# justinkay/coda

Measured on NVIDIA H100. Metric: acquisition steps/sec (M=256,N=5e5,C=100), higher is better.
Workload: dtype f32

## Files before the change

coda_b200/_native.py:

```python
from __future__ import annotations

import ctypes as C
import os
import sys

from . import build as _build

_LIB = None

OK = 0
VERSION = 202
MAX_WORLD = 16
REC_WORDS = 8
FLAG_NONFINITE_INPUT = 0x01
FLAG_RANGE_INPUT = 0x02
FLAG_NONFINITE_TABLE = 0x04
FLAG_NONFINITE_PI = 0x08
FLAG_NONFINITE_PBEST = 0x10
FLAG_NONFINITE_EIG = 0x20
FLAG_NO_CANDIDATE = 0x40
FLAG_XCHG_TIMEOUT = 0x80
FLAG_NEGATIVE_PROB = 0x100
FLAG_ROWSUM_WARN = 0x200
FLAG_PIPELINE_TIMEOUT = 0x400
# ... 36 lines not shown

PX, PS = C.POINTER(XchgStruct), C.POINTER(StepStruct)

SIGNATURES = {
    "coda_b200_last_error": (C.c_char_p, []),
    "coda_b200_version": (i32, []),
    "coda_b200_sm_count": (i32, []),
    "coda_b200_device_check": (i32, []),
    "coda_b200_set_l2_fetch_granularity": (i32, [i32]),
    "coda_b200_xchg_box_bytes": (sz, [i32, i32, i32, i32]),
    "coda_b200_xchg_alloc": (i32, [sz, C.POINTER(p)]),
    "coda_b200_xchg_free": (i32, [p]),
    "coda_b200_ipc_export": (i32, [p, p]),
    "coda_b200_ipc_open": (i32, [p, C.POINTER(p)]),
    "coda_b200_ipc_close": (i32, [p]),
    "coda_b200_peer_enable": (i32, [i32]),
    "coda_b200_scan_slab": (i32, [p, i64, i32, i64, i32, p, p, p, p, p, p]),
    "coda_b200_confusion_accum": (i32, [p, i64, p, i32, i64, i32, i32, p, p]),
    "coda_b200_confusion_sorted": (i32, [p, i64, p, p, i32, i64, i32, i32, p, p]),
    "coda_b200_init_dirichlets": (i32, [p, p, i32, i32, i32, f64, f64, i32, p, p]),
    "coda_b200_scan_compact": (i32, [p, p, i64, i32, i64, i32, i32, p, p, p, p, p, p]),
    "coda_b200_confusion_compact": (i32, [p, p, i64, p, i32, i64, i32, i32, i32, p, p, p]),
    "coda_b200_pi_full_compact": (i32, [p, p, i64, p, i32, i64, i32, i32, p, p, p, p]),
    "coda_b200_pi_rank1_compact": (i32, [p, p, i64, p, i32, i64, i32, i32, p, f64, i32, p, p, p, p, p]),
    "coda_b200_compact_index_count": (i32, [p, i64, i32, i64, i32, i32, p, p]),
    "coda_b200_compact_index_fill": (i32, [p, p, i64, i32, i64, i32, i32, p, p, p, p]),
    "coda_b200_pi_rank1_index": (i32, [p, p, p, p, i32, i64, i32, p, f64, i32, p, p, p, p, p, p]),
    "coda_b200_pi_full": (i32, [p, i64, p, i32, i64, i32, p, p]),
    "coda_b200_pi_full_tc_ok": (i32, [i32, i64, i32, i64]),
    "coda_b200_pi_full_tc_scratch_bytes": (sz, [i32, i32]),
    "coda_b200_pi_full_tc": (i32, [p, i64, p, i32, i64, i32, p, p, p, p]),
    "coda_b200_pi_reduce": (i32, [p, i64, i32, i32, p, p, p, p]),
    "coda_b200_shadow_build": (i32, [p, i64, i32, i64, i32, p, i32, i64, p, p]),
    "coda_b200_pi_rank1": (i32, [p, p, i32, i64, i32, p, f64, i32, p, p, p, p, i32, i32, p]),
    "coda_b200_scan_slab_x": (i32, [p, i32, i64, i32, i64, i32, p, p, p, p, p, p]),
    "coda_b200_confusion_accum_x": (i32, [p, i32, i64, p, i32, i64, i32, i32, p, p]),
    "coda_b200_confusion_sorted_x": (i32, [p, i32, i64, p, p, i32, i64, i32, i32, p, p]),
    "coda_b200_pi_full_x": (i32, [p, i32, i64, p, i32, i64, i32, p, p]),
    "coda_b200_pi_full_tc_ok_x": (i32, [i32, i32, i64, i32, i64]),
    "coda_b200_pi_full_tc_x": (i32, [p, i32, i64, p, i32, i64, i32, p, p, p, p]),
    "coda_b200_shadow_build_x": (i32, [p, i32, i64, i32, i64, i32, p, i32, i64, p, p]),
    "coda_b200_pi_rank1_x": (i32, [p, i32, p, i32, i64, i32, p, f64, i32, p, p, p, p, i32, i32, p]),
    "coda_b200_tables_scratch_bytes": (sz, [i32, i32]),
    "coda_b200_beta_tables": (i32, [p, p, i32, i32, i32, f64, i32, i32, p, p, p, p, p, p, p, p, p, p]),
    "coda_b200_pair_count": (i32, [p, i32, i64, i32, p, p, p, p]),
    "coda_b200_pair_fill": (i32, [p, i32, i64, i32, p, p, p, p, p, p, p, p, p, p]),
    "coda_b200_pair_rows": (i32, [p, i32, i32, p, p, p, p, p, p, p, p, i32, p, p, p, p, p, p]),
    "coda_b200_pair_rows_tc": (i32, [p, i32, i32, p, p, p, p, p, p, p, i32, p, p, p, p, p, p]),
    "coda_b200_template_gains": (i32, [p, i32, i32, p, p, p, p, p]),
    "coda_b200_eig_blocks": (i32, [i64, i32, i32]),
    "coda_b200_gain_eig": (i32, [p, i64, i32, i32, p, p, p, p, p, p, p, p, p, p, p, i64, i32, p, p, i32, p, p, p, p]),
    "coda_b200_ell_build": (i32, [p, p, p, i64, i32, p, p, p]),
    "coda_b200_row_gains": (i32, [p, p, i64, i32, i32, p, p, p, p, p]),
    "coda_b200_step_select": (i32, [PS, PX, p]),
    "coda_b200_step_merge": (i32, [PS, PX, p]),
    "coda_b200_step_label": (i32, [PS, PX, p]),
    "coda_b200_step_mixture": (i32, [PS, PX, p]),
    "coda_b200_ties": (i32, [p, i64, p, p, i64, p, i32, p, p, p, p]),
    "coda_b200_report_gather": (i32, [p, i32, p, PX, p, p]),
    "coda_b200_mp_entropy": (i32, [p, p, i32, i64, i32, f64, p, p, i32, p, p]),
    "coda_b200_static_scores": (i32, [p, p, i32, i64, i32, p, p, p]),
    "coda_b200_select_blocks": (i32, [i64]),
    "coda_b200_weighted_total": (i32, [p, p, i64, p, p, p]),
    "coda_b200_weighted_draw": (i32, [p, p, i64, p, f64, p, p, p]),
    "coda_b200_select_extreme": (i32, [p, p, i64, i32, p, p, p]),
    "coda_b200_select_kth": (i32, [p, p, i64, p, p, i64, p, p]),
}


class NativeError(RuntimeError):
    pass


def lib_path() -> str:
    return _build.LIB


def load(build_if_missing: bool = True):
    global _LIB
    if _LIB is not None:
        return _LIB
    path = lib_path()
    if build_if_missing and not os.environ.get("CODA_B200_NO_BUILD"):
        try:
            _build.build()
        except Exception as e:
            if not os.path.exists(path):
                raise NativeError(f"cannot build {path}: {e}") from e
            if not _build.is_fresh():
                raise NativeError(f"{path} was built from different sources (build.sha256 does not match csrc/ and "
                                  f"include/) and rebuilding failed: {e}") from e
    if not os.path.exists(path):
        raise NativeError(f"{path} is missing; run `python -m coda_b200.build`")
    if os.environ.get("CODA_B200_NO_BUILD") and not _build.is_fresh():
        sys.stderr.write(f"coda_b200: WARNING: {path} does not match the current sources (CODA_B200_NO_BUILD is set)\n")
    lib = C.CDLL(path)
    for name, (res, args) in SIGNATURES.items():
        fn = getattr(lib, name)
        fn.restype = res
        fn.argtypes = args
    if lib.coda_b200_version() != VERSION:
        raise NativeError(f"{path} reports ABI version {lib.coda_b200_version()}, this binding expects {VERSION}")
    _LIB = lib
    return lib


# ... 16 lines not shown
```

coda_b200/csrc/gain.cu:

```cuda
#include "common.cuh"

#include <stdlib.h>

#define GE_THREADS 384
#define GE_WARPS (GE_THREADS / 32)

struct GainEigArgs {
  const float* U;
  long long N;
  int C, H, Hp, T;
  const int32_t* ent_off;
  const int32_t* heavy_off;
  const int32_t* ent_row;
  const uint16_t* ent_cls;
  const float* ph_cache;
  const float* gain;
  const float* PB;
  const float* m0;
  const float* pi_hat;
  const uint8_t* labeled;
  const uint8_t* disagree;
  long long n_offset;
  float* eig;
  long long* partials;
// ... 179 lines not shown
      for (int k = 0; k < KR; ++k) {
        const int c = lane + 32 * k;
        s += u[k];
        if (c < C) e = fmaf(u[k], g0[c], e);
      }
    } else {
      for (int c = lane; c < C; c += 32) {
        const float v = __ldg(urow + c);
        s += v;
        e = fmaf(v, g0[c], e);
      }
    }
    s = warp_sum(s);
    e = warp_sum(e);
    if (lane == 0) {
      const float v = e / fmaxf(s, 1e-12f);
      a.eig[n] = v;
      if (!isfinite(v)) bad |= CODA_B200_FLAG_NONFINITE_EIG;
      if (!a.labeled[n]) {
        best2_add(bB, v, a.n_offset + n);
        if (a.disagree[n]) {
          best2_add(bA, v, a.n_offset + n);
          ++cntA;
        }
      }
    }
    n = nn; e0 = ne0; e1 = ne1; h0 = nh0; h1 = nh1;
  }
  if (lane == 0) {
    s_v[0][warp] = bA.v; s_i[0][warp] = bA.i; s_v2[0][warp] = bA.v2;
    s_v[1][warp] = bB.v; s_i[1][warp] = bB.i; s_v2[1][warp] = bB.v2;
    s_c[warp] = cntA;
  }
  __syncthreads();
  if (tid == 0) {
    Best2 fa = best2_empty(), fb = best2_empty();
    long long cn = 0;
    for (int w = 0; w < GE_WARPS; ++w) {
      best2_merge(fa, Best2{s_v[0][w], s_i[0][w], s_v2[0][w]});
      best2_merge(fb, Best2{s_v[1][w], s_i[1][w], s_v2[1][w]});
      cn += s_c[w];
    }
    rec_store(a.partials + (size_t)blockIdx.x * REC_W, fa, cn, fb);
  }
  if (bad) atomicOr(a.flags, bad);
}

__device__ __forceinline__ float4 ld_stream4(const float4* p) {
  float4 v;
  asm volatile("ld.global.cs.v4.f32 {%0, %1, %2, %3}, [%4];" : "=f"(v.x), "=f"(v.y), "=f"(v.z), "=f"(v.w) : "l"(p));
  return v;
}

template <int NQ>
__global__ void __launch_bounds__(256) k_row_gains(const float* __restrict__ rows, const uint16_t* __restrict__ row_cls,
                                                   long long nrows, long long T, int H, const float* __restrict__ PB,
                                                   const float* __restrict__ m0, const float* __restrict__ pi_hat,
                                                   float* __restrict__ gain) {
  constexpr int Hp = 128 * NQ;
  constexpr int CH = 32;
  const int warp = threadIdx.x >> 5, lane = threadIdx.x & 31;
  float4 m[NQ], fm[NQ];
#pragma unroll
  for (int q = 0; q < NQ; ++q) {
    const int h = (q * 32 + lane) * 4;
    float4 v = __ldg(reinterpret_cast<const float4*>(m0) + q * 32 + lane);
    if (h + 0 >= H) v.x = 0.f;
    if (h + 1 >= H) v.y = 0.f;
    if (h + 2 >= H) v.z = 0.f;
    if (h + 3 >= H) v.w = 0.f;
    m[q] = v;
    fm[q] = make_float4(ent_term(v.x), ent_term(v.y), ent_term(v.z), ent_term(v.w));
  }
  const long long nchunks = (nrows + CH - 1) / CH;
  for (long long ch = (long long)blockIdx.x * 8 + warp; ch < nchunks; ch += (long long)gridDim.x * 8) {
    const long long p0 = ch * CH;
    const long long p1 = min(nrows, p0 + CH);
    int mycls = 0;
    if (p0 + lane < p1) mycls = (p0 + lane < T) ? (int)((p0 + lane) / (1 + H)) : (int)row_cls[p0 + lane - T];
    for (long long i = p0; i < p1; i += 4) {
      float4 a[4][NQ];
#pragma unroll
      for (int j = 0; j < 4; ++j) {
        const long long r = min(i + j, nrows - 1);
        const float4* rp = reinterpret_cast<const float4*>(rows + (size_t)r * Hp);
#pragma unroll
        for (int q = 0; q < NQ; ++q) a[j][q] = ld_stream4(rp + q * 32 + lane);
      }
#pragma unroll
      for (int j = 0; j < 4; ++j) {
        const long long r = i + j;
        if (r < p1) {
          const int c = __shfl_sync(CODA_FULL, mycls, (int)(r - p0));
          const float pic = __ldg(pi_hat + c);
          const float4* pb = reinterpret_cast<const float4*>(PB + (size_t)c * Hp);
          float g = 0.f;
#pragma unroll
          for (int q = 0; q < NQ; ++q) g += gain4(a[j][q], __ldg(pb + q * 32 + lane), m[q], fm[q], pic);
          g = warp_sum(g);
          if (lane == 0) gain[r] = g;
        }
      }
    }
  }
}

__global__ void __launch_bounds__(256) k_row_gains_any(const float* __restrict__ rows, const uint16_t* __restrict__ row_cls,
                                                       long long nrows, long long T, int H, int Hp, const float* __restrict__ PB,
                                                       const float* __restrict__ m0, const float* __restrict__ pi_hat,
                                                       float* __restrict__ gain) {
  extern __shared__ __align__(16) unsigned char smem_raw[];
  float* m0s = reinterpret_cast<float*>(smem_raw);
  float* fm0 = m0s + Hp;
  for (int h = threadIdx.x; h < Hp; h += blockDim.x) {
    const float m = h < H ? m0[h] : 0.f;
    m0s[h] = m;
    fm0[h] = ent_term(m);
  }
  __syncthreads();
  const int warp = threadIdx.x >> 5, lane = threadIdx.x & 31;
  for (long long r = (long long)blockIdx.x * 8 + warp; r < nrows; r += (long long)gridDim.x * 8) {
    const int c = r < T ? (int)(r / (1 + H)) : (int)row_cls[r - T];
    const float pic = pi_hat[c];
    const float* row = rows + (size_t)r * Hp;
    const float* pb = PB + (size_t)c * Hp;
    float g = 0.f;
    for (int hq = lane * 4; hq < Hp; hq += 128) {
      const float4 ph = ld_stream4(reinterpret_cast<const float4*>(row + hq));
      const float4 p4 = __ldg(reinterpret_cast<const float4*>(pb + hq));
      const float4 m4 = *reinterpret_cast<const float4*>(m0s + hq);
      const float4 f4 = *reinterpret_cast<const float4*>(fm0 + hq);
      g += gain4(ph, p4, m4, f4, pic);
    }
    g = warp_sum(g);
    if (lane == 0) gain[r] = g;
  }
}

extern "C" int coda_b200_row_gains(const float* ph_cache, const uint16_t* row_cls, int64_t n_heavy, int H, int C,
                                   const float* PB, const float* m0, const float* pi_hat, float* gain,
                                   coda_stream_t stream) {
  CODA_CHECK_ARG(ph_cache && PB && m0 && pi_hat && gain && (row_cls || n_heavy == 0), "row_gains: null pointer");
  const int Hp = (H + 31) / 32 * 32;
  const long long T = (long long)C * (1 + H);
  const long long nrows = T + (n_heavy > 0 ? n_heavy : 0);
  const float* rows = ph_cache;
  float* g = gain;
  cudaStream_t st = as_stream(stream);
  if (Hp % 128 == 0 && Hp <= 512) {
    int grid = (int)min((long long)(nrows + 255) / 256, (long long)coda_sm_count() * 6);
    if (grid < 1) grid = 1;
#define LAUNCH_RG(NQ) k_row_gains<NQ><<<grid, 256, 0, st>>>(rows, row_cls, nrows, T, H, PB, m0, pi_hat, g)
    if (Hp == 128) LAUNCH_RG(1);
    else if (Hp == 256) LAUNCH_RG(2);
    else if (Hp == 384) LAUNCH_RG(3);
    else LAUNCH_RG(4);
#undef LAUNCH_RG
    CODA_LAUNCH_OK("k_row_gains");
    return CODA_B200_OK;
  }
  int grid = (int)min((long long)(nrows + 7) / 8, (long long)coda_sm_count() * 8);
  if (grid < 1) grid = 1;
  k_row_gains_any<<<grid, 256, (size_t)2 * Hp * 4, st>>>(rows, row_cls, nrows, T, H, Hp, PB, m0, pi_hat, g);
  CODA_LAUNCH_OK("k_row_gains_any");
  return CODA_B200_OK;
}

template <int KC8, int IT8>
__global__ void __launch_bounds__(256, (IT8 == 1 ? 3 : 2)) k_eig_assemble_g8(GainEigArgs a, int nblocks_rec) {
  extern __shared__ __align__(16) unsigned char smem_raw[];
  float* g0 = reinterpret_cast<float*>(smem_raw);
  __shared__ float s_v[2][8], s_v2[2][8];
  __shared__ long long s_i[2][8], s_c[8];
  const int C = a.C;
  for (int c = threadIdx.x; c < C; c += blockDim.x) g0[c] = a.gain[(size_t)c * (1 + a.H)];
  __syncthreads();
  const int warp = threadIdx.x >> 5, lane = threadIdx.x & 31, g = lane & 7, grp = lane >> 3;
  Best2 bA = best2_empty(), bB = best2_empty();
  long long cntA = 0;
  uint32_t bad = 0;
  const long long per_iter = (long long)gridDim.x * 8 * 4 * IT8;
  for (long long wb = ((long long)blockIdx.x * 8 + warp) * 4 * IT8; wb < a.N; wb += per_iter) {
    const long long nb = wb + grp * IT8;
    int e0[IT8], ne[IT8];
    if (!a.ell_row) {
#pragma unroll
      for (int i = 0; i < IT8; ++i) {
        const long long n = min(nb + i, a.N - 1);
        e0[i] = __ldg(a.ent_off + n);
        ne[i] = __ldg(a.ent_off + n + 1) - e0[i];
      }
    }
    float u[IT8][KC8];
    int er[IT8][4], ec[IT8][4];
#pragma unroll
    for (int i = 0; i < IT8; ++i) {
      const long long n = min(nb + i, a.N - 1);
      const float* urow = a.U + (size_t)n * C;
#pragma unroll
      for (int k = 0; k < KC8; ++k) {
        const int c = g + 8 * k;
        u[i][k] = c < C ? __ldg(urow + c) : 0.f;
      }
#pragma unroll
      for (int j = 0; j < 4; ++j) {
        const int e = g + 8 * j;
        er[i][j] = -1; ec[i][j] = 0;
        if (a.ell_row) {
          if (e < a.ell_k) {
            er[i][j] = __ldg(a.ell_row + (size_t)n * a.ell_k + e);
            ec[i][j] = __ldg(a.ell_cls + (size_t)n * a.ell_k + e);
          }
        } else if (e < ne[i]) {
          er[i][j] = __ldg(a.ent_row + e0[i] + e);
          ec[i][j] = __ldg(a.ent_cls + e0[i] + e);
        }
      }
    }
// ... 222 lines not shown
```

coda_b200/csrc/step.cu:

```cuda
#include "xchg.cuh"
#include "terms.cuh"

#define ST_THREADS 256

__device__ void apply_label(const coda_step_t& a, int t, const int* jv, int* cnt , bool valid) {
  const int H = a.H, C = a.C, tid = threadIdx.x;
  unsigned long long* pz = reinterpret_cast<unsigned long long*>(a.pisum_fx);
  for (int c = tid; c < C; c += ST_THREADS) pz[c] = 0ull;
  int32_t* hdr = a.terms;
  R1Term* terms = reinterpret_cast<R1Term*>(a.terms + 2);
  if (!valid) {
    if (tid == 0) { hdr[0] = 0; hdr[1] = -1; }
    return;
  }
  for (int h = tid; h < H; h += ST_THREADS) {
    a.jvec[h] = jv[h];
    a.D[((size_t)h * C + t) * C + jv[h]] += a.lr;
  }
  __shared__ int s_tp, s_m, s_total;
  __shared__ int wtot[ST_THREADS / 32];
  for (int c = tid; c < C; c += ST_THREADS) cnt[c] = 0;
  __syncthreads();
  for (int h = tid; h < H; h += ST_THREADS) atomicAdd(&cnt[jv[h]], 1);
  __syncthreads();
// ... 317 lines not shown
  if (x.world > 1) xch_done(x, XCH_PISUM, ep);
}

static int check_step(const coda_step_t* st, const char* who) {
  CODA_CHECK_ARG(st, "%s: null state", who);
  CODA_CHECK_ARG(st->H >= 1 && st->H <= 1024 && st->C >= 2 && st->C <= 4096 && st->N >= 1, "%s: bad dims", who);
  CODA_CHECK_ARG(st->flags, "%s: flags missing", who);
  return CODA_B200_OK;
}

static size_t select_smem(int H, int C) { return 64 + 2 * (size_t)xch_align16((uint32_t)H * 2) + (size_t)H * 4 + (size_t)C * 4; }

static int launch_select(const coda_step_t* st, const coda_xchg_t* x, int pick, coda_stream_t stream) {
  if (int rc = check_step(st, "step_select")) return rc;
  CODA_CHECK_ARG(st->partials && st->nblocks >= 1 && st->bestrec, "step_select: selection buffers missing");
  if (pick) {
    CODA_CHECK_ARG(st->hard && st->labeled && st->D && st->jvec && st->sel && st->terms && st->pisum_fx && st->labels_global &&
                       st->step_ctr,
                   "step_select: null pointer");
    CODA_CHECK_ARG(2 * st->H <= R1_MAXT && (reinterpret_cast<uintptr_t>(st->terms) & 7) == 0, "step_select: bad terms buffer");
  }
  XchgView v;
  if (int rc = xchg_view_from(x, &v)) return rc;
  k_step_select<<<1, ST_THREADS, select_smem(st->H, st->C), as_stream(stream)>>>(*st, v, pick);
  CODA_LAUNCH_OK("k_step_select");
  return CODA_B200_OK;
}

extern "C" int coda_b200_step_select(const coda_step_t* st, const coda_xchg_t* x, coda_stream_t stream) {
  return launch_select(st, x, 1, stream);
}
extern "C" int coda_b200_step_merge(const coda_step_t* st, const coda_xchg_t* x, coda_stream_t stream) {
  return launch_select(st, x, 0, stream);
}

extern "C" int coda_b200_step_label(const coda_step_t* st, const coda_xchg_t* x, coda_stream_t stream) {
  if (int rc = check_step(st, "step_label")) return rc;
  CODA_CHECK_ARG(st->hard && st->labeled && st->D && st->jvec && st->sel && st->terms && st->pisum_fx, "step_label: null pointer");
  CODA_CHECK_ARG(2 * st->H <= R1_MAXT && (reinterpret_cast<uintptr_t>(st->terms) & 7) == 0, "step_label: bad terms buffer");
  XchgView v;
  if (int rc = xchg_view_from(x, &v)) return rc;
  const size_t smem = 16 + (size_t)xch_align16((uint32_t)st->H * 2) + (size_t)st->H * 4 + (size_t)st->C * 4;
  k_step_label<<<1, ST_THREADS, smem, as_stream(stream)>>>(*st, v);
  CODA_LAUNCH_OK("k_step_label");
  return CODA_B200_OK;
}

extern "C" int coda_b200_step_mixture(const coda_step_t* st, const coda_xchg_t* x, coda_stream_t stream) {
  if (int rc = check_step(st, "step_mixture")) return rc;
  CODA_CHECK_ARG(st->pisum_fx && st->PB && st->pi_hat && st->m0 && st->h_before && st->best_model, "step_mixture: null pointer");
  XchgView v;
  if (int rc = xchg_view_from(x, &v)) return rc;
  const size_t smem = (size_t)xch_align16((uint32_t)st->C * 8) + (size_t)st->C * 4;
  k_step_mixture<<<1, ST_THREADS, smem, as_stream(stream)>>>(*st, v);
  CODA_LAUNCH_OK("k_step_mixture");
  return CODA_B200_OK;
}

__global__ void __launch_bounds__(256) k_ties(const float* __restrict__ eig, long long N,
                                              const uint8_t* __restrict__ labeled,
                                              const uint8_t* __restrict__ disagree, long long n_offset,
                                              const long long* __restrict__ best, int cap,
                                              long long* __restrict__ tie_hdr, long long* __restrict__ tie_idx,
                                              float* __restrict__ tie_val) {
  const bool useA = best[2] > 0;
  const float bv = __int_as_float((int)(useA ? best[0] : best[3]));
  for (long long n = (long long)blockIdx.x * blockDim.x + threadIdx.x; n < N;
       n += (long long)gridDim.x * blockDim.x) {
    if (labeled[n]) continue;
    if (useA && !disagree[n]) continue;
    const float e = eig[n];
    if (isclose_best(e, bv)) {
      const long long g = n_offset + n;
      unsigned long long k = atomicAdd(reinterpret_cast<unsigned long long*>(tie_hdr), 1ull);
      atomicMin(tie_hdr + 1, g);
      if (k < (unsigned long long)cap) {
        tie_idx[k] = g;
        tie_val[k] = e;
      }
    }
  }
}

__global__ void k_ties_reset(long long* tie_hdr) {
  tie_hdr[0] = 0;
  tie_hdr[1] = IDX_NONE;
}

extern "C" int coda_b200_ties(const float* eig, int64_t N, const uint8_t* labeled, const uint8_t* disagree,
                              int64_t n_offset, const int64_t* best, int cap, int64_t* tie_hdr, int64_t* tie_idx,
                              float* tie_val, coda_stream_t stream) {
  CODA_CHECK_ARG(eig && labeled && disagree && best && tie_hdr && tie_idx && tie_val, "ties: null pointer");
  int grid = (int)min((long long)(N + 255) / 256, (long long)coda_sm_count() * 4);
  if (grid < 1) grid = 1;
  k_ties_reset<<<1, 1, 0, as_stream(stream)>>>(reinterpret_cast<long long*>(tie_hdr));
  k_ties<<<grid, 256, 0, as_stream(stream)>>>(eig, N, labeled, disagree, n_offset,
                                              reinterpret_cast<const long long*>(best), cap,
                                              reinterpret_cast<long long*>(tie_hdr),
                                              reinterpret_cast<long long*>(tie_idx), tie_val);
  CODA_LAUNCH_OK("k_ties");
  return CODA_B200_OK;
}

__global__ void __launch_bounds__(ST_THREADS) k_report_gather(const long long* __restrict__ rep, int rep_words,
                                                              long long* __restrict__ rep_all, XchgView x,
                                                              uint32_t* __restrict__ flags) {
  if (x.world <= 1) {
// ... 28 lines not shown
```

coda_b200/engine.py:

```python
from __future__ import annotations

import contextlib
import math
import os

import numpy as np
import torch

from . import _native as nat

_CONST_SLOTS = {}
_CONST_TERMS = 3584


def _acquire_const_slot(dev_index, H):
    per = (2 * H + 63) // 64 * 64
    used = _CONST_SLOTS.setdefault(dev_index, set())
    for s in range(_CONST_TERMS // per):
        if s not in used:
            used.add(s)
            return s
    return -1


# ... 64 lines not shown
        self.Hp = (H + 31) // 32 * 32
        self.W = self.Hp // 32
        self.P = 256
        self.T = Cc * (1 + H)
        self.mode = mode
        self.world = int(world)
        self.n_offset = int(n_offset)
        self.n_global = int(n_global if n_global is not None else N)
        self.lr = float(learning_rate)
        self.hyp_w = float(hyp_w)
        self.prior_strength = 1 - alpha
        self.multiplier = float(multiplier)
        self.uniform_prior = bool(uniform_prior)
        if H > 1024:
            raise NotImplementedError("coda_b200: H > 1024 models is not supported yet")
        if Cc > 4096:
            raise NotImplementedError("coda_b200: C > 4096 classes is not supported yet")
        self.fx_shift = max(8, min(40, 62 - math.ceil(math.log2(self.n_global + 1))))
        self.counters = {"launches": 0}
        self.overlap = os.environ.get("CODA_B200_OVERLAP", "1") != "0"
        self.use_graph = os.environ.get("CODA_B200_GRAPH", "1") != "0"
        self.profile, self.profile_only = None, None
        self.xchg = None
        self._mailbox = None
        self._pi_tc, self._pi_scratch = None, None
        self.cidx = None
        self.stream = torch.cuda.Stream(device=self.dev) if own_stream else None
        self.side = torch.cuda.Stream(device=self.dev)
        self.ev_fork, self.ev_join, self.ev_tables = torch.cuda.Event(), torch.cuda.Event(), torch.cuda.Event()
        self.graphs = {}
        self.labels_ptr = None
        self.const_slot = _acquire_const_slot(self.dev.index, H) if os.environ.get("CODA_B200_R1_CONST", "1") != "0" else -1
        with self._on():
            self._alloc_static()

    @contextlib.contextmanager
    def _on(self):
        with torch.cuda.device(self.dev):
            if self.stream is not None:
                with torch.cuda.stream(self.stream):
                    yield
            else:
                yield

    def _cur(self):
        return torch.cuda.current_stream(self.dev)

    def _s(self):
        return self._cur().cuda_stream

    def sync(self):
        (self.stream or torch.cuda.current_stream(self.dev)).synchronize()

    def _call(self, name, *args, n=1):
        prof = self.profile
        key = name[:-2] if name.endswith("_x") else name
        if prof is not None and (self.profile_only is None or key in self.profile_only):
            st = self._cur()
            e0, e1 = torch.cuda.Event(enable_timing=True), torch.cuda.Event(enable_timing=True)
            e0.record(st)
            rc = getattr(self.lib, name)(*args)
            e1.record(st)
            prof.setdefault(key, []).append((e0, e1))
        else:
            rc = getattr(self.lib, name)(*args)
        nat.check(rc, name)
        self.counters["launches"] += n

    def start_profile(self, only=None):
        self.profile, self.profile_only = {}, (set(only) if only else None)

    def stop_profile(self):
        torch.cuda.synchronize(self.dev)
        out = {}
        for k, v in (self.profile or {}).items():
            ts = [a.elapsed_time(b) for a, b in v]
            out[k] = (len(ts), float(sum(ts)), float(max(ts)))
        self.profile = None
        return out

    def _slab_call(self, name, *args, n=1):
        if self.fmt == nat.SLAB_F32:
            self._call(name, _ptr(self.preds), *args, n=n)
        else:
            self._call(name + "_x", _ptr(self.preds), self.fmt, *args, n=n)

    def _z(self, shape, dtype):
        return torch.zeros(shape, dtype=dtype, device=self.dev)

    def _e(self, shape, dtype):
        return torch.empty(shape, dtype=dtype, device=self.dev)

    def _alloc_static(self):
        H, N, C, Hp, P = self.H, self.N, self.C, self.Hp, self.P
        self.hard = self._e((N, H), torch.int16)
        self.pseudo = self._e((N,), torch.int32)
        self.disagree = self._e((N,), torch.uint8)
        self.labeled = self._z((N,), torch.uint8)
        self.conf_buf = self._z((H * C * C + H * C,), torch.int64)
        self.conf_fx = self.conf_buf[: H * C * C].view(H, C, C)
        self.conf_rest = self.conf_buf[H * C * C:].view(H, C) if self.compact is not None else None
        self.D = self._e((H, C, C), torch.float32)
        self.U = self._e((N * C + 4,), torch.float32)[: N * C].view(N, C)
        self.pisum = self._z((C,), torch.int64)
        self.grid = torch.linspace(1e-6, 1 - 1e-6, P).to(self.dev)
        self.dL = self._e((C, H, P), torch.float32)
        self.G0T = self._z((C, P, Hp), torch.float32)
        self.G1T = self._z((C, P, Hp), torch.float32)
        self.PB = self._z((C, Hp), torch.float32)
# ... 149 lines not shown
                       self.K, _ptr(dt), _ptr(rs), _ptr(self.U), s, n=3)
            del dt, rs
        else:
            self._pi_full()
        self._call("coda_b200_pi_reduce", _ptr(self.U), N, C, self.fx_shift, None, _ptr(self.pisum),
                   _ptr(self.flags), s)

    def _pi_full(self):
        H, N, C, s = self.H, self.N, self.C, self._s()
        if self._pi_tc is None:
            want = os.environ.get("CODA_B200_PI_FULL", "tc") != "simt"
            if self.fmt == nat.SLAB_F32:
                self._pi_tc = bool(want and self.lib.coda_b200_pi_full_tc_ok(H, N, C, self.model_stride)
                                   and self.preds.data_ptr() % 16 == 0)
            else:
                tc32 = bool(self.lib.coda_b200_pi_full_tc_ok(H, N, C, N * C))
                ok = bool(self.lib.coda_b200_pi_full_tc_ok_x(self.fmt, H, N, C, self.model_stride))
                if want and tc32 and not ok:
                    raise NotImplementedError(f"coda_b200: the tensor-core marginal pass cannot read this "
                                              f"{self.preds.dtype} slab (C={C}); its fp32 widening would take it")
                self._pi_tc = bool(want and tc32)
            if self._pi_tc:
                self._pi_scratch = self._e((int(self.lib.coda_b200_pi_full_tc_scratch_bytes(H, C)),), torch.uint8)
        if self._pi_tc:
            self._slab_call("coda_b200_pi_full_tc", self.model_stride, _ptr(self.D), H, N, C, _ptr(self.U),
                            _ptr(self._pi_scratch), _ptr(self.flags), s, n=2)
        else:
            self._slab_call("coda_b200_pi_full", self.model_stride, _ptr(self.D), H, N, C, _ptr(self.U), s)

    def _build_rows(self):
        H, N, C, W, T, s = self.H, self.N, self.C, self.W, self.T, self._s()
        ent_cnt = self._e((N,), torch.int32)
        heavy_cnt = self._e((N,), torch.int32)
        cls_heavy = self._z((C,), torch.int32)
        self._call("coda_b200_pair_count", _ptr(self.hard), H, N, C, _ptr(ent_cnt), _ptr(heavy_cnt), _ptr(cls_heavy), s)
        heavy = cls_heavy.cpu().numpy().astype(np.int64)
        n_ent = int(ent_cnt.sum(dtype=torch.int64).item())
        self.n_heavy = int(heavy.sum())
        self.n_entries = n_ent
        self.max_entries = int(ent_cnt.max().item())
        per_cls = 1 + H + heavy
        cls_base = np.zeros(C + 1, dtype=np.int64)
        np.cumsum(per_cls, out=cls_base[1:])
        self.npairs = int(cls_base[-1])
        if self.npairs >= 2 ** 31 or n_ent >= 2 ** 31:
            raise NotImplementedError("coda_b200: more than 2^31 rows in one shard")
        self.ent_off = self._z((N + 1,), torch.int32)
        self.heavy_off = self._z((N + 1,), torch.int32)
        torch.cumsum(ent_cnt, 0, out=self.ent_off[1:])
        torch.cumsum(heavy_cnt, 0, out=self.heavy_off[1:])
        del ent_cnt, heavy_cnt
        self.cls_base_host = cls_base
        self.cls_base = torch.from_numpy(cls_base).to(self.dev)
        def make_tiles(width):
            nt = (per_cls + width - 1) // width
            tile_off = np.zeros(C + 1, dtype=np.int64)
            np.cumsum(nt, out=tile_off[1:])
            cls_of_tile = np.repeat(np.arange(C, dtype=np.int64), nt)
            k_in_cls = np.arange(int(tile_off[-1]), dtype=np.int64) - tile_off[cls_of_tile]
            start = cls_base[cls_of_tile] + width * k_in_cls
            cnt = np.minimum(width, per_cls[cls_of_tile] - width * k_in_cls)
            tiles = np.stack([cls_of_tile, start, cnt, np.zeros_like(cnt)], axis=1).astype(np.int32)
            return tile_off, int(nt.max()), torch.from_numpy(tiles).to(self.dev)
        width = 128 if self.use_tc else 32
        tile_off, self.max_cls_tiles, self.tiles = make_tiles(width)
        self.tile_off_host = tile_off
        self.tile_off = torch.from_numpy(tile_off).to(self.dev)
        self.ntiles = int(tile_off[-1])
        self.ent_row = self._e((max(1, n_ent),), torch.int32)
        self.ent_cls = self._e((max(1, n_ent),), torch.int16)
        self.zmask = self._e((self.npairs, W), torch.int32)
        self.row_of = self._e((self.npairs,), torch.int32)
        self.row_cls = self._e((max(1, self.n_heavy),), torch.int16)
        cursor = self._z((C,), torch.int32)
        self._call("coda_b200_pair_fill", _ptr(self.hard), H, N, C, _ptr(self.ent_off), _ptr(self.heavy_off),
                   _ptr(self.cls_base), _ptr(cursor), _ptr(self.ent_row), _ptr(self.ent_cls), _ptr(self.zmask),
                   _ptr(self.row_of), _ptr(self.row_cls), s, n=2)
        self.ell_row, self.ell_cls, self.ell_k = None, None, 0
        if 0 < self.max_entries <= 32 and C <= 128:
            self.ell_k = (self.max_entries + 3) // 4 * 4
            self.ell_row = self._e((N, self.ell_k), torch.int32)
            self.ell_cls = self._e((N, self.ell_k), torch.int16)
            self._call("coda_b200_ell_build", _ptr(self.ent_off), _ptr(self.ent_row), _ptr(self.ent_cls), N, self.ell_k,
                       _ptr(self.ell_row), _ptr(self.ell_cls), s)
        self.gain = self._z((self.npairs,), torch.float32)
        self.fused_score = os.environ.get("CODA_B200_FUSED_SCORE", "0") == "1"
        self.ph_cache = None
        if self.mode == "incremental":
            need = self.npairs * self.Hp * 4
            free, _total = torch.cuda.mem_get_info(self.dev)
            if need + (2 << 30) > free + torch.cuda.memory_reserved(self.dev) - torch.cuda.memory_allocated(self.dev):
                import warnings
                warnings.warn(f"coda_b200: row cache of {need / 2 ** 30:.1f} GiB does not fit "
                              f"({free / 2 ** 30:.1f} GiB free); falling back to mode='recompute'")
                self.mode = "recompute"
            else:
                self.ph_cache = self._e((self.npairs, self.Hp), torch.float32)

    def shadow_reserve(self) -> int:
        env = os.environ.get("CODA_B200_SHADOW_RESERVE_GB")
        if env is not None:
            return int(float(env) * 2 ** 30)
        return 4 * self.N * self.C + (1 << 30)

    def _build_shadow(self, left: int = 1, total: int = 1):
        self.shadow, self.slot_of_model, self.n_shadow, self.shadow_cs = None, None, 0, 0
# ... 22 lines not shown
            return
        slot = torch.full((H,), -1, dtype=torch.int32, device=self.dev)
        if self.esz == 4:
            self.shadow = self._e((S + ne, C, cs), torch.float32)
            self.ens_shadow = self.shadow[S] if ne else None
        else:
            self.shadow = self._e((S, C, cs), self.preds.dtype) if S > 0 else None
            self.ens_shadow = self._e((C, cs), torch.float32) if ne else None
        if S > 0:
            order = order[:S].contiguous()
            slot[order.long()] = torch.arange(S, dtype=torch.int32, device=self.dev)
            self._slab_call("coda_b200_shadow_build", self.model_stride, H, N, C, _ptr(order), S, cs,
                            _ptr(self.shadow), self._s())
        if ne:
            first = torch.zeros(1, dtype=torch.int32, device=self.dev)
            self._call("coda_b200_shadow_build", _ptr(self.ens), N * C, 1, N, C, _ptr(first), 1, cs,
                       _ptr(self.ens_shadow), self._s())
        self.slot_of_model, self.n_shadow, self.shadow_cs = slot, S, cs

    def _tables(self, lo, hi, sel=False):
        H, C, s = self.H, self.C, self._s()
        if sel:
            self._call("coda_b200_beta_tables", _ptr(self.D), _ptr(self.grid), H, C, self.P, self.hyp_w, 0, 1,
                       _ptr(self.sel), _ptr(self.scratch), _ptr(self.dL), _ptr(self.G0T), _ptr(self.G1T),
                       _ptr(self.PB), _ptr(self.dLb), _ptr(self.Gb), _ptr(self.flags), s, n=3)
            return
        for b0 in range(lo, hi, self.table_batch):
            b1 = min(hi, b0 + self.table_batch)
            self._call("coda_b200_beta_tables", _ptr(self.D), _ptr(self.grid), H, C, self.P, self.hyp_w, b0, b1, None,
                       _ptr(self.scratch), _ptr(self.dL), _ptr(self.G0T), _ptr(self.G1T), _ptr(self.PB),
                       _ptr(self.dLb), _ptr(self.Gb), _ptr(self.flags), s, n=3)

    def _mixture(self):
        self._call("coda_b200_step_mixture", self.st, self._x(), self._s())

    def _pair_rows(self, tile_lo, tile_hi, gains=True, sel=False):
        tail = (_ptr(self.PB), _ptr(self.m0) if gains else None, _ptr(self.pi_hat) if gains else None, self.H,
                _ptr(self.ph_cache), _ptr(self.gain) if gains else None, _ptr(self.sel) if sel else None,
                _ptr(self.tile_off) if sel else None, _ptr(self.flags), self._s())
        if self.use_tc:
            self._call("coda_b200_pair_rows_tc", _ptr(self.tiles), int(tile_lo), int(tile_hi), _ptr(self.zmask),
                       _ptr(self.row_of), _ptr(self.dLb), _ptr(self.Gb), *tail)
        else:
            self._call("coda_b200_pair_rows", _ptr(self.tiles), int(tile_lo), int(tile_hi), _ptr(self.zmask),
                       _ptr(self.row_of), _ptr(self.dL), _ptr(self.G0T), _ptr(self.G1T), *tail)

    def _score(self):
        if self.scored:
            return
        if self.mode == "incremental":
            if not self.cache_valid:
                self._pair_rows(0, self.ntiles, gains=False)
                self.cache_valid = True
            if self.pending:
                self._cur().wait_event(self.ev_join)
                self.pending = False
            if self.fused_score:
                self._call("coda_b200_template_gains", _ptr(self.ph_cache), self.H, self.C, _ptr(self.PB), _ptr(self.m0),
                           _ptr(self.pi_hat), _ptr(self.gain), self._s())
            else:
                self._call("coda_b200_row_gains", _ptr(self.ph_cache), _ptr(self.row_cls), self.n_heavy, self.H, self.C,
                           _ptr(self.PB), _ptr(self.m0), _ptr(self.pi_hat), _ptr(self.gain), self._s())
        else:
            if self.pending:
                self._cur().wait_event(self.ev_join)
                self.pending = False
            self._pair_rows(0, self.ntiles)
        self._call("coda_b200_gain_eig", _ptr(self.U), self.N, self.C, self.H, _ptr(self.ent_off), _ptr(self.heavy_off),
                   _ptr(self.ent_row), _ptr(self.ent_cls), _ptr(self.ph_cache) if self.fused_score else None,
                   _ptr(self.gain), _ptr(self.PB), _ptr(self.m0), _ptr(self.pi_hat), _ptr(self.labeled),
                   _ptr(self.disagree), self.n_offset, self.max_entries, _ptr(self.ell_row), _ptr(self.ell_cls),
                   self.ell_k, _ptr(self.eig), _ptr(self.partials), _ptr(self.flags), self._s())
        self.scored = True

    def _post_label(self):
        H, N, C, s = self.H, self.N, self.C, self._s()
        self.scored = False
        self.reported = False
        if self.mode == "recompute_all":
            self._pi_full()
            self._call("coda_b200_pi_reduce", _ptr(self.U), N, C, self.fx_shift, None, _ptr(self.pisum), _ptr(self.flags), s)
            self._tables(0, C)
            self._mixture()
            return
        main = self._cur()
        refresh_rows = self.mode == "incremental" and self.cache_valid
        fork = self.overlap
        if fork:
            self.ev_fork.record(main)
            self.side.wait_event(self.ev_fork)
            ctx = torch.cuda.stream(self.side)
        else:
            ctx = contextlib.nullcontext()
        with ctx:
            self._tables(0, 1, sel=True)
            if fork:
                self.ev_tables.record(self.side)
            if refresh_rows:
                self._pair_rows(0, self.max_cls_tiles, gains=False, sel=True)
            if fork:
                self.ev_join.record(self.side)
        if self.compact is not None and self.cidx is not None:
            ix = self.cidx
            self._call("coda_b200_pi_rank1_index", _ptr(ix["off"]), _ptr(ix["ent"]), _ptr(ix["rest"]), _ptr(self.jvec), H, N, C,
                       _ptr(self.sel), self.lr, self.fx_shift, _ptr(self.terms), _ptr(ix["delta"]), _ptr(self.U),
                       _ptr(self.pisum), _ptr(self.flags), s, n=2)
        elif self.compact is not None:
            cs = self.compact
            self._call("coda_b200_pi_rank1_compact", _ptr(cs.ids), _ptr(cs.probs), self.model_stride, _ptr(self.ens), H, N,
                       C, self.K, _ptr(self.sel), self.lr, self.fx_shift, _ptr(self.terms), _ptr(self.U),
                       _ptr(self.pisum), _ptr(self.flags), s)
        else:
            ens = _ptr(self.ens) if self.fmt == nat.SLAB_F32 else self._ens_base()
            self._slab_call("coda_b200_pi_rank1", ens, H, N, C, _ptr(self.sel), self.lr,
                            self.fx_shift, _ptr(self.terms), _ptr(self.U), _ptr(self.pisum), _ptr(self.flags),
# ... 279 lines not shown
```

include/coda_b200.h:

```cpp
#ifndef CODA_B200_H
#define CODA_B200_H

#include <stddef.h>
#include <stdint.h>

#ifdef __cplusplus
extern "C" {
#endif

#define CODA_B200_VERSION 202
#define CODA_B200_NODES 256
#define CODA_B200_MAX_WORLD 16
#define CODA_B200_REC_WORDS 8

#define CODA_B200_OK 0
#define CODA_B200_EINVAL (-1)
#define CODA_B200_ECUDA (-2)

#define CODA_B200_FLAG_NONFINITE_INPUT 0x01u
#define CODA_B200_FLAG_RANGE_INPUT 0x02u
#define CODA_B200_FLAG_NONFINITE_TABLE 0x04u
#define CODA_B200_FLAG_NONFINITE_PI 0x08u
#define CODA_B200_FLAG_NONFINITE_PBEST 0x10u
#define CODA_B200_FLAG_NONFINITE_EIG 0x20u
// ... 87 lines not shown
                                int H, int64_t N, int C, int K, int fx_shift, int64_t* conf_fx, int64_t* conf_rest,
                                coda_stream_t stream);
int coda_b200_pi_full_compact(const uint16_t* ids, const float* probs, int64_t model_stride, const float* D, int H,
                              int64_t N, int C, int K, float* DT_scratch, float* RS_scratch, float* U,
                              coda_stream_t stream);
int coda_b200_pi_rank1_compact(const uint16_t* ids, const float* probs, int64_t model_stride, const float* ens, int H,
                               int64_t N, int C, int K, const int64_t* sel, double lr, int fx_shift,
                               const int32_t* terms, float* U, int64_t* pisum_fx, uint32_t* flags,
                               coda_stream_t stream);

int coda_b200_compact_index_count(const uint16_t* ids, int64_t model_stride, int H, int64_t N, int C, int K,
                                  int64_t* counts, coda_stream_t stream);
int coda_b200_compact_index_fill(const uint16_t* ids, const float* probs, int64_t model_stride, int H, int64_t N, int C,
                                 int K, int64_t* cursor, void* entries, float* rest_sum, coda_stream_t stream);
int coda_b200_pi_rank1_index(const int64_t* offsets, const void* entries, const float* rest_sum, const int32_t* jvec,
                             int H, int64_t N, int C, const int64_t* sel, double lr, int fx_shift, const int32_t* terms,
                             int64_t* delta, float* U, int64_t* pisum_fx, uint32_t* flags, coda_stream_t stream);

size_t coda_b200_tables_scratch_bytes(int H, int ncls);
int coda_b200_beta_tables(const float* D, const float* grid_x, int H, int C, int P, double hyp_w, int cls_lo,
                          int cls_hi, const int64_t* sel, void* scratch, float* dL ,
                          float* G0T , float* G1T , float* PB , void* dLb,
                          void* Gb, uint32_t* flags, coda_stream_t stream);

int coda_b200_pair_count(const uint16_t* hard, int H, int64_t N, int C, int32_t* ent_cnt ,
                         int32_t* heavy_cnt , int32_t* cls_heavy , coda_stream_t stream);
int coda_b200_pair_fill(const uint16_t* hard, int H, int64_t N, int C, const int32_t* ent_off ,
                        const int32_t* heavy_off , const int64_t* cls_base ,
                        int32_t* cls_cursor , int32_t* ent_row, uint16_t* ent_cls,
                        uint32_t* zmask , int32_t* row_of ,
                        uint16_t* row_cls , coda_stream_t stream);
int coda_b200_pair_rows(const int32_t* tiles, int tile_lo, int tile_hi, const uint32_t* zmask, const int32_t* row_of,
                        const float* dL, const float* G0T, const float* G1T, const float* PB, const float* m0,
                        const float* pi_hat, int H, float* ph_cache, float* gain, const int64_t* sel ,
                        const int64_t* tile_off , uint32_t* flags, coda_stream_t stream);
int coda_b200_pair_rows_tc(const int32_t* tiles128, int tile_lo, int tile_hi, const uint32_t* zmask,
                           const int32_t* row_of, const void* dLb, const void* Gb, const float* PB, const float* m0,
                           const float* pi_hat, int H, float* ph_cache, float* gain, const int64_t* sel,
                           const int64_t* tile_off, uint32_t* flags, coda_stream_t stream);
int coda_b200_template_gains(const float* ph_cache, int H, int C, const float* PB, const float* m0,
                             const float* pi_hat, float* gain , coda_stream_t stream);

int coda_b200_eig_blocks(int64_t N, int H, int C);
int coda_b200_gain_eig(const float* U, int64_t N, int C, int H, const int32_t* ent_off, const int32_t* heavy_off,
                       const int32_t* ent_row, const uint16_t* ent_cls, const float* ph_cache, const float* gain,
                       const float* PB, const float* m0, const float* pi_hat, const uint8_t* labeled,
                       const uint8_t* disagree, int64_t n_offset, int max_entries, const int32_t* ell_row,
                       const uint16_t* ell_cls, int ell_k, float* eig, int64_t* partials, uint32_t* flags,
                       coda_stream_t stream);
int coda_b200_ell_build(const int32_t* ent_off, const int32_t* ent_row, const uint16_t* ent_cls, int64_t N, int K,
                        int32_t* ell_row , uint16_t* ell_cls , coda_stream_t stream);
int coda_b200_row_gains(const float* ph_cache, const uint16_t* row_cls, int64_t n_heavy, int H, int C,
                        const float* PB, const float* m0, const float* pi_hat, float* gain, coda_stream_t stream);

typedef struct coda_step {
  int H, C;
  int64_t N, n_offset;
  int fx_shift;
  float lr;
  const uint16_t* hard;
  uint8_t* labeled;
  float* D;
  int32_t* jvec;
  int64_t* sel;
  int32_t* terms;
  const int32_t* slot_of_model;
  int64_t shadow_off, shadow_col_stride, model_stride;
  int64_t ens_off, ens_col_stride;
  int have_ens;
  int compact_k;
  int64_t* pisum_fx;
  const float* PB;
  float* pi_hat;
  float* m0;
  float* h_before;
  int64_t* best_model;
  const int64_t* partials;
  int nblocks;
  const float* eig;
  int64_t* bestrec;
  const int64_t* labels_global;
  int64_t* hist_idx;
  float* hist_q;
  int32_t* hist_tie;
  int64_t hist_cap;
  int64_t* step_ctr;
  uint32_t* flags;
} coda_step_t;

int coda_b200_step_select(const coda_step_t* st, const coda_xchg_t* x, coda_stream_t stream);
int coda_b200_step_merge(const coda_step_t* st, const coda_xchg_t* x, coda_stream_t stream);
int coda_b200_step_label(const coda_step_t* st, const coda_xchg_t* x, coda_stream_t stream);
int coda_b200_step_mixture(const coda_step_t* st, const coda_xchg_t* x, coda_stream_t stream);

int coda_b200_ties(const float* eig, int64_t N, const uint8_t* labeled, const uint8_t* disagree, int64_t n_offset,
                   const int64_t* best , int cap, int64_t* tie_hdr , int64_t* tie_idx,
                   float* tie_val, coda_stream_t stream);
int coda_b200_report_gather(const int64_t* rep, int rep_words, int64_t* rep_all, const coda_xchg_t* x,
                            uint32_t* flags, coda_stream_t stream);


int coda_b200_mp_entropy(const uint16_t* hard, const float* posterior , int H, int64_t N, int C, double gamma,
                         const uint8_t* labeled, const uint8_t* disagree, int mask_agreeing, float* ent,
                         coda_stream_t stream);
int coda_b200_static_scores(const uint16_t* hard, const float* ens, int H, int64_t N, int C, float* at_score,
                            float* vma_score, coda_stream_t stream);
// ... 15 lines not shown
```

Before: 661.0.

## Split row gains so unaffected classes compute before the pending pair-row join

Row-gain scoring is split into two launches. The first covers every class except the one just labelled and runs before waiting on the side-stream join event. After the join, a second launch recomputes only the labelled class's rows through a row_of/cls_base index. This lets most of the gain work overlap the pending pair-row refresh instead of waiting for it, at the cost of an extra launch and indirect row addressing. The mixture kernel is also launched with high stream priority via cudaLaunchKernelEx, and the grid sizing for the vectorized row kernel now scales with span rather than being capped by SM count.

```diff
diff --git a/coda_b200/_native.py b/coda_b200/_native.py
--- a/coda_b200/_native.py
+++ b/coda_b200/_native.py
@@ -112,6 +112,8 @@
     "coda_b200_gain_eig": (i32, [p, i64, i32, i32, p, p, p, p, p, p, p, p, p, p, p, i64, i32, p, p, i32, p, p, p, p]),
     "coda_b200_ell_build": (i32, [p, p, p, i64, i32, p, p, p]),
     "coda_b200_row_gains": (i32, [p, p, i64, i32, i32, p, p, p, p, p]),
+    "coda_b200_row_gains_except": (i32, [p, p, i64, i32, i32, p, p, p, p, p, p]),
+    "coda_b200_row_gains_class": (i32, [p, p, p, i64, i32, i32, p, p, p, p, p, p]),
     "coda_b200_step_select": (i32, [PS, PX, p]),
     "coda_b200_step_merge": (i32, [PS, PX, p]),
     "coda_b200_step_label": (i32, [PS, PX, p]),
diff --git a/coda_b200/csrc/gain.cu b/coda_b200/csrc/gain.cu
--- a/coda_b200/csrc/gain.cu
+++ b/coda_b200/csrc/gain.cu
@@ -255,14 +255,33 @@
   return v;
 }
 
+struct RowSet {
+  const long long* sel;
+  const int32_t* row_of;
+  const long long* cls_base;
+};
+
+__device__ __forceinline__ void row_set_range(const RowSet& s, long long nrows, long long& p_lo, long long& p_hi,
+                                              int& skip, int& t) {
+  p_lo = 0; p_hi = nrows; skip = -1; t = 0;
+  if (s.sel) {
+    t = (int)s.sel[1];
+    if (s.row_of) { p_lo = s.cls_base[t]; p_hi = s.cls_base[t + 1]; }
+    else skip = t;
+  }
+}
+
 template <int NQ>
 __global__ void __launch_bounds__(256) k_row_gains(const float* __restrict__ rows, const uint16_t* __restrict__ row_cls,
                                                    long long nrows, long long T, int H, const float* __restrict__ PB,
                                                    const float* __restrict__ m0, const float* __restrict__ pi_hat,
-                                                   float* __restrict__ gain) {
+                                                   RowSet rs, float* __restrict__ gain) {
   constexpr int Hp = 128 * NQ;
   constexpr int CH = 32;
   const int warp = threadIdx.x >> 5, lane = threadIdx.x & 31;
+  long long p_lo, p_hi;
+  int skip, t;
+  row_set_range(rs, nrows, p_lo, p_hi, skip, t);
   float4 m[NQ], fm[NQ];
 #pragma unroll
   for (int q = 0; q < NQ; ++q) {
@@ -275,26 +294,42 @@
     m[q] = v;
     fm[q] = make_float4(ent_term(v.x), ent_term(v.y), ent_term(v.z), ent_term(v.w));
   }
-  const long long nchunks = (nrows + CH - 1) / CH;
+  const long long nchunks = (p_hi - p_lo + CH - 1) / CH;
   for (long long ch = (long long)blockIdx.x * 8 + warp; ch < nchunks; ch += (long long)gridDim.x * 8) {
-    const long long p0 = ch * CH;
-    const long long p1 = min(nrows, p0 + CH);
-    int mycls = 0;
-    if (p0 + lane < p1) mycls = (p0 + lane < T) ? (int)((p0 + lane) / (1 + H)) : (int)row_cls[p0 + lane - T];
-    for (long long i = p0; i < p1; i += 4) {
+    const long long p0 = p_lo + ch * CH;
+    const long long p1 = min(p_hi, p0 + CH);
+    int myrow = (int)(p0 + lane);
+    int mycls = t;
+    if (p0 + lane < p1) {
+      if (rs.row_of) myrow = rs.row_of[p0 + lane];
+      else mycls = (p0 + lane < T) ? (int)((p0 + lane) / (1 + H)) : (int)row_cls[p0 + lane - T];
+    }
+    const int n = (int)(p1 - p0);
+    for (int i = 0; i < n; i += 4) {
       float4 a[4][NQ];
+      int rj[4], cj[4];
 #pragma unroll
       for (int j = 0; j < 4; ++j) {
-        const long long r = min(i + j, nrows - 1);
-        const float4* rp = reinterpret_cast<const float4*>(rows + (size_t)r * Hp);
-#pragma unroll
-        for (int q = 0; q < NQ; ++q) a[j][q] = ld_stream4(rp + q * 32 + lane);
+        const int l = min(i + j, n - 1);
+        rj[j] = __shfl_sync(CODA_FULL, myrow, l);
+        cj[j] = __shfl_sync(CODA_FULL, mycls, l);
       }
 #pragma unroll
       for (int j = 0; j < 4; ++j) {
-        const long long r = i + j;
-        if (r < p1) {
-          const int c = __shfl_sync(CODA_FULL, mycls, (int)(r - p0));
+        const float4* rp = reinterpret_cast<const float4*>(rows + (size_t)rj[j] * Hp);
+        if (cj[j] != skip) {
+#pragma unroll
+          for (int q = 0; q < NQ; ++q) a[j][q] = ld_stream4(rp + q * 32 + lane);
+        } else {
+#pragma unroll
+          for (int q = 0; q < NQ; ++q) a[j][q] = make_float4(0.f, 0.f, 0.f, 0.f);
+        }
+      }
+#pragma unroll
+      for (int j = 0; j < 4; ++j) {
+        const int r = rj[j];
+        if (i + j < n && cj[j] != skip) {
+          const int c = cj[j];
           const float pic = __ldg(pi_hat + c);
           const float4* pb = reinterpret_cast<const float4*>(PB + (size_t)c * Hp);
           float g = 0.f;
@@ -311,7 +346,7 @@
 __global__ void __launch_bounds__(256) k_row_gains_any(const float* __restrict__ rows, const uint16_t* __restrict__ row_cls,
                                                        long long nrows, long long T, int H, int Hp, const float* __restrict__ PB,
                                                        const float* __restrict__ m0, const float* __restrict__ pi_hat,
-                                                       float* __restrict__ gain) {
+                                                       RowSet rs, float* __restrict__ gain) {
   extern __shared__ __align__(16) unsigned char smem_raw[];
   float* m0s = reinterpret_cast<float*>(smem_raw);
   float* fm0 = m0s + Hp;
@@ -321,9 +356,14 @@
     fm0[h] = ent_term(m);
   }
   __syncthreads();
+  long long p_lo, p_hi;
+  int skip, t;
+  row_set_range(rs, nrows, p_lo, p_hi, skip, t);
   const int warp = threadIdx.x >> 5, lane = threadIdx.x & 31;
-  for (long long r = (long long)blockIdx.x * 8 + warp; r < nrows; r += (long long)gridDim.x * 8) {
-    const int c = r < T ? (int)(r / (1 + H)) : (int)row_cls[r - T];
+  for (long long p = p_lo + (long long)blockIdx.x * 8 + warp; p < p_hi; p += (long long)gridDim.x * 8) {
+    const long long r = rs.row_of ? (long long)rs.row_of[p] : p;
+    const int c = rs.row_of ? t : (r < T ? (int)(r / (1 + H)) : (int)row_cls[r - T]);
+    if (c == skip) continue;
     const float pic = pi_hat[c];
     const float* row = rows + (size_t)r * Hp;
     const float* pb = PB + (size_t)c * Hp;
@@ -340,10 +380,9 @@
   }
 }
 
-extern "C" int coda_b200_row_gains(const float* ph_cache, const uint16_t* row_cls, int64_t n_heavy, int H, int C,
-                                   const float* PB, const float* m0, const float* pi_hat, float* gain,
-                                   coda_stream_t stream) {
-  CODA_CHECK_ARG(ph_cache && PB && m0 && pi_hat && gain && (row_cls || n_heavy == 0), "row_gains: null pointer");
+static int row_gains_launch(const float* ph_cache, const uint16_t* row_cls, int64_t n_heavy, int H, int C,
+                            const float* PB, const float* m0, const float* pi_hat, RowSet rs, long long span,
+                            float* gain, coda_stream_t stream) {
   const int Hp = (H + 31) / 32 * 32;
   const long long T = (long long)C * (1 + H);
   const long long nrows = T + (n_heavy > 0 ? n_heavy : 0);
@@ -351,9 +390,9 @@
   float* g = gain;
   cudaStream_t st = as_stream(stream);
   if (Hp % 128 == 0 && Hp <= 512) {
-    int grid = (int)min((long long)(nrows + 255) / 256, (long long)coda_sm_count() * 6);
+    int grid = (int)((span + 255) / 256);
     if (grid < 1) grid = 1;
-#define LAUNCH_RG(NQ) k_row_gains<NQ><<<grid, 256, 0, st>>>(rows, row_cls, nrows, T, H, PB, m0, pi_hat, g)
+#define LAUNCH_RG(NQ) k_row_gains<NQ><<<grid, 256, 0, st>>>(rows, row_cls, nrows, T, H, PB, m0, pi_hat, rs, g)
     if (Hp == 128) LAUNCH_RG(1);
     else if (Hp == 256) LAUNCH_RG(2);
     else if (Hp == 384) LAUNCH_RG(3);
@@ -362,11 +401,41 @@
     CODA_LAUNCH_OK("k_row_gains");
     return CODA_B200_OK;
   }
-  int grid = (int)min((long long)(nrows + 7) / 8, (long long)coda_sm_count() * 8);
+  int grid = (int)min((long long)(span + 7) / 8, (long long)coda_sm_count() * 8);
   if (grid < 1) grid = 1;
-  k_row_gains_any<<<grid, 256, (size_t)2 * Hp * 4, st>>>(rows, row_cls, nrows, T, H, Hp, PB, m0, pi_hat, g);
+  k_row_gains_any<<<grid, 256, (size_t)2 * Hp * 4, st>>>(rows, row_cls, nrows, T, H, Hp, PB, m0, pi_hat, rs, g);
   CODA_LAUNCH_OK("k_row_gains_any");
   return CODA_B200_OK;
+}
+
+extern "C" int coda_b200_row_gains(const float* ph_cache, const uint16_t* row_cls, int64_t n_heavy, int H, int C,
+                                   const float* PB, const float* m0, const float* pi_hat, float* gain,
+                                   coda_stream_t stream) {
+  CODA_CHECK_ARG(ph_cache && PB && m0 && pi_hat && gain && (row_cls || n_heavy == 0), "row_gains: null pointer");
+  const long long nrows = (long long)C * (1 + H) + (n_heavy > 0 ? n_heavy : 0);
+  return row_gains_launch(ph_cache, row_cls, n_heavy, H, C, PB, m0, pi_hat, RowSet{nullptr, nullptr, nullptr}, nrows,
+                          gain, stream);
+}
+
+extern "C" int coda_b200_row_gains_except(const float* ph_cache, const uint16_t* row_cls, int64_t n_heavy, int H,
+                                          int C, const float* PB, const float* m0, const float* pi_hat,
+                                          const int64_t* sel, float* gain, coda_stream_t stream) {
+  CODA_CHECK_ARG(ph_cache && PB && m0 && pi_hat && gain && sel && (row_cls || n_heavy == 0),
+                 "row_gains_except: null pointer");
+  const long long nrows = (long long)C * (1 + H) + (n_heavy > 0 ? n_heavy : 0);
+  return row_gains_launch(ph_cache, row_cls, n_heavy, H, C, PB, m0, pi_hat,
+                          RowSet{reinterpret_cast<const long long*>(sel), nullptr, nullptr}, nrows, gain, stream);
+}
+
+extern "C" int coda_b200_row_gains_class(const float* ph_cache, const int32_t* row_of, const int64_t* cls_base,
+                                         int64_t max_cls_rows, int H, int C, const float* PB, const float* m0,
+                                         const float* pi_hat, const int64_t* sel, float* gain, coda_stream_t stream) {
+  CODA_CHECK_ARG(ph_cache && row_of && cls_base && PB && m0 && pi_hat && gain && sel, "row_gains_class: null pointer");
+  CODA_CHECK_ARG(max_cls_rows >= 1, "row_gains_class: max_cls_rows=%lld", (long long)max_cls_rows);
+  return row_gains_launch(ph_cache, nullptr, 0, H, C, PB, m0, pi_hat,
+                          RowSet{reinterpret_cast<const long long*>(sel), row_of,
+                                 reinterpret_cast<const long long*>(cls_base)},
+                          max_cls_rows, gain, stream);
 }
 
 template <int KC8, int IT8>
diff --git a/coda_b200/csrc/step.cu b/coda_b200/csrc/step.cu
--- a/coda_b200/csrc/step.cu
+++ b/coda_b200/csrc/step.cu
@@ -393,7 +393,19 @@
   XchgView v;
   if (int rc = xchg_view_from(x, &v)) return rc;
   const size_t smem = (size_t)xch_align16((uint32_t)st->C * 8) + (size_t)st->C * 4;
-  k_step_mixture<<<1, ST_THREADS, smem, as_stream(stream)>>>(*st, v);
+  int prio_lo = 0, prio_hi = 0;
+  CODA_CUDA_OK(cudaDeviceGetStreamPriorityRange(&prio_lo, &prio_hi));
+  cudaLaunchAttribute at[1];
+  at[0].id = cudaLaunchAttributePriority;
+  at[0].val.priority = prio_hi;
+  cudaLaunchConfig_t cfg = {};
+  cfg.gridDim = dim3(1);
+  cfg.blockDim = dim3(ST_THREADS);
+  cfg.dynamicSmemBytes = smem;
+  cfg.stream = as_stream(stream);
+  cfg.attrs = at;
+  cfg.numAttrs = 1;
+  CODA_CUDA_OK(cudaLaunchKernelEx(&cfg, k_step_mixture, *st, v));
   CODA_LAUNCH_OK("k_step_mixture");
   return CODA_B200_OK;
 }
diff --git a/coda_b200/engine.py b/coda_b200/engine.py
--- a/coda_b200/engine.py
+++ b/coda_b200/engine.py
@@ -140,9 +140,10 @@
     def sync(self):
         (self.stream or torch.cuda.current_stream(self.dev)).synchronize()
 
-    def _call(self, name, *args, n=1):
+    def _call(self, name, *args, n=1, key=None):
         prof = self.profile
-        key = name[:-2] if name.endswith("_x") else name
+        if key is None:
+            key = name[:-2] if name.endswith("_x") else name
         if prof is not None and (self.profile_only is None or key in self.profile_only):
             st = self._cur()
             e0, e1 = torch.cuda.Event(enable_timing=True), torch.cuda.Event(enable_timing=True)
@@ -398,6 +399,8 @@
         del ent_cnt, heavy_cnt
         self.cls_base_host = cls_base
         self.cls_base = torch.from_numpy(cls_base).to(self.dev)
+        self.max_cls_rows = int(per_cls.max())
+        self.split_gains = self.n_heavy <= 8 * N
         def make_tiles(width):
             nt = (per_cls + width - 1) // width
             tile_off = np.zeros(C + 1, dtype=np.int64)
@@ -526,15 +529,24 @@
             if not self.cache_valid:
                 self._pair_rows(0, self.ntiles, gains=False)
                 self.cache_valid = True
-            if self.pending:
+            gain_args = (_ptr(self.PB), _ptr(self.m0), _ptr(self.pi_hat))
+            if self.pending and self.split_gains and not self.fused_score:
+                self._call("coda_b200_row_gains_except", _ptr(self.ph_cache), _ptr(self.row_cls), self.n_heavy, self.H,
+                           self.C, *gain_args, _ptr(self.sel), _ptr(self.gain), self._s(), key="coda_b200_row_gains")
                 self._cur().wait_event(self.ev_join)
                 self.pending = False
-            if self.fused_score:
-                self._call("coda_b200_template_gains", _ptr(self.ph_cache), self.H, self.C, _ptr(self.PB), _ptr(self.m0),
-                           _ptr(self.pi_hat), _ptr(self.gain), self._s())
+                self._call("coda_b200_row_gains_class", _ptr(self.ph_cache), _ptr(self.row_of), _ptr(self.cls_base),
+                           self.max_cls_rows, self.H, self.C, *gain_args, _ptr(self.sel), _ptr(self.gain), self._s())
             else:
-                self._call("coda_b200_row_gains", _ptr(self.ph_cache), _ptr(self.row_cls), self.n_heavy, self.H, self.C,
-                           _ptr(self.PB), _ptr(self.m0), _ptr(self.pi_hat), _ptr(self.gain), self._s())
+                if self.pending:
+                    self._cur().wait_event(self.ev_join)
+                    self.pending = False
+                if self.fused_score:
+                    self._call("coda_b200_template_gains", _ptr(self.ph_cache), self.H, self.C, *gain_args,
+                               _ptr(self.gain), self._s())
+                else:
+                    self._call("coda_b200_row_gains", _ptr(self.ph_cache), _ptr(self.row_cls), self.n_heavy, self.H,
+                               self.C, *gain_args, _ptr(self.gain), self._s())
         else:
             if self.pending:
                 self._cur().wait_event(self.ev_join)
diff --git a/include/coda_b200.h b/include/coda_b200.h
--- a/include/coda_b200.h
+++ b/include/coda_b200.h
@@ -163,6 +163,12 @@
                         int32_t* ell_row , uint16_t* ell_cls , coda_stream_t stream);
 int coda_b200_row_gains(const float* ph_cache, const uint16_t* row_cls, int64_t n_heavy, int H, int C,
                         const float* PB, const float* m0, const float* pi_hat, float* gain, coda_stream_t stream);
+int coda_b200_row_gains_except(const float* ph_cache, const uint16_t* row_cls, int64_t n_heavy, int H, int C,
+                               const float* PB, const float* m0, const float* pi_hat, const int64_t* sel, float* gain,
+                               coda_stream_t stream);
+int coda_b200_row_gains_class(const float* ph_cache, const int32_t* row_of, const int64_t* cls_base ,
+                              int64_t max_cls_rows, int H, int C, const float* PB, const float* m0,
+                              const float* pi_hat, const int64_t* sel, float* gain, coda_stream_t stream);
 
 typedef struct coda_step {
   int H, C;
```

Result: faster. 679.2 (median of 6 runs) (+2.7%).
